# ldyken53/gaussian-splatting-wgpu

Hardware: AMD Instinct MI355X
Metric: frames/sec (higher is better)
Workload: dtype f32; 1 GPU; bicycle-like synthetic 6.1M gaussians @1920x1080; gaussians=6100000, width=1920, height=1080, tile_size=16, parallelism=single GPU, visible=2430918, processed=15909895, block_evaluated=6068168, sort_passes=1, depth_ordered_emission=True, tight_binning=True, blend_mode=fused, camera=64-step orbit, moved every frame

## Files before the change

### gaussian-splatting-wgpu_amd/csrc/k_blend.hip

```cpp
#include "gs_device.h"
#include "gs_tight.h"
#include <type_traits>

__device__ __forceinline__ float block_qmin(float cx, float cy, float cz, float dxlo, float dxhi, float dylo, float dyhi,
                                            float& mag) {
    const float X = __builtin_fminf(__builtin_fmaxf(0.0f, dxlo), dxhi);
    const float Y = __builtin_fminf(__builtin_fmaxf(0.0f, dylo), dyhi);
    float q = 3.0e38f;
    mag = 0.0f;
    if (X == 0.0f && Y == 0.0f) return 0.0f;
    if (X != 0.0f) {
        const float dy = __builtin_fminf(__builtin_fmaxf(-cy * X * __builtin_amdgcn_rcpf(cz), dylo), dyhi);
        const float a = 0.5f * cx * X * X, b = 0.5f * cz * dy * dy, c = cy * X * dy;
        q = a + b + c;
        mag = __builtin_fabsf(a) + __builtin_fabsf(b) + __builtin_fabsf(c);
    }
    if (Y != 0.0f) {
        const float dx = __builtin_fminf(__builtin_fmaxf(-cy * Y * __builtin_amdgcn_rcpf(cx), dxlo), dxhi);
        const float a = 0.5f * cx * dx * dx, b = 0.5f * cz * Y * Y, c = cy * dx * Y;
        const float q2 = a + b + c;
        if (q2 < q) { q = q2; mag = __builtin_fabsf(a) + __builtin_fabsf(b) + __builtin_fabsf(c); }
    }
    return q;
}

__device__ __forceinline__ bool blend_tmax_cull(float cx, float cy, float cz, float op, float dxlo, float dxhi, float dylo, float dyhi, float Tmax) {
    const float ax0 = (0.5f * cx) * dxlo * dxlo, ax1 = (0.5f * cx) * dxhi * dxhi, by0 = (0.5f * cz) * dylo * dylo, by1 = (0.5f * cz) * dyhi * dyhi;
    const float c00 = cy * dxlo * dylo, c01 = cy * dxlo * dyhi, c10 = cy * dxhi * dylo, c11 = cy * dxhi * dyhi;
    const float qmax = __builtin_fmaxf(__builtin_fmaxf(ax0 + by0 + c00, ax0 + by1 + c01), __builtin_fmaxf(ax1 + by0 + c10, ax1 + by1 + c11));
    const float qmag = __builtin_fmaxf(ax0, ax1) + __builtin_fmaxf(by0, by1) +
                       __builtin_fmaxf(__builtin_fmaxf(__builtin_fabsf(c00), __builtin_fabsf(c01)), __builtin_fmaxf(__builtin_fabsf(c10), __builtin_fabsf(c11)));
    const float alo = 0.99f * __builtin_fminf(0.99f, op * __builtin_amdgcn_exp2f(-1.44269502162933349609375f * (qmax + 1.0e-5f * qmag)));
    return Tmax * (1.0f - alo) < 0.0000999f;
}

struct GsAuxPlanes { float* alpha; float* depth; };
__device__ __forceinline__ GsAuxPlanes gs_aux_planes() { return GsAuxPlanes{nullptr, nullptr}; }
__device__ __forceinline__ GsAuxPlanes gs_aux_planes(GsAuxPlanes p) { return p; }

template <int TS, bool EXACT, bool AUX = false, typename... Aux>
__global__ __launch_bounds__(TS* TS) void gs_blend_kernel(const uint4* __restrict__ gdata, const uint32_t* __restrict__ values,
                                                           const uint32_t* __restrict__ ranges, GsFrame f,
                                                           uint32_t* __restrict__ rgba8, float* __restrict__ rgbf, GsControl* ctl,
                                                           uint32_t dbg, uint32_t id_mask, Aux... aux) {
    static_assert(sizeof...(Aux) == (AUX ? 1u : 0u), "AUX kernels take one GsAuxPlanes, the others none");
    constexpr int NT = TS * TS;
    constexpr int ROUNDS = NT / 64;
    constexpr int WPR = TS / 8;
    __shared__ float4 sP0[2][NT];
    __shared__ float4 sP1[2][NT];
    __shared__ float4 sP2[2][NT];

    const uint32_t tid = threadIdx.x, lane = tid & 63, w = tid >> 6;
    const uint32_t tx = f.col0 + blockIdx.x, ty = blockIdx.y;
    const uint32_t tile = tx + ty * f.ntx;
    const uint32_t start = tile > 0 ? ranges[tile - 1] : 0u;
    uint32_t end = ranges[tile];
    if (end > f.capacity) end = f.capacity;

    const uint32_t bx0 = tx * TS + (w % WPR) * 8, by0 = ty * TS + (w / WPR) * 8;
    const uint32_t gx = bx0 + (lane & 7), gy = by0 + (lane >> 3);
    const float pxf = (float)gx, pyf = (float)gy;
    const float bx0f = (float)bx0, by0f = (float)by0;
    float T = 1.0f, cr = 0.0f, cg = 0.0f, cb = 0.0f;
    float cd = 0.0f;
    const bool outside = !(gx < f.width && gy < f.height);
    bool done = outside;
    const float c255 = (float)(1.0 / 255.0);
    const float Wf = (float)f.width, Hf = (float)f.height;
    uint32_t staged = 0, evaluated = 0;

    const uint32_t piece = lane & 3u, qrec = lane >> 2;
    uint4 rq[4];
    uint32_t gnext = 0;
    auto fetch_ids = [&](uint32_t b) { gnext = (b + tid < end) ? values[b + tid] : 0u; };
    auto fetch = [&](uint32_t b, uint32_t gval) {
#pragma unroll
        for (int i = 0; i < 4; ++i) {
            const uint32_t rec = qrec + 16u * i;
            uint32_t g = __shfl(gval, rec, 64) & id_mask;
#ifdef GS_PROFILING
            if (dbg & 2u) g &= 1023u;
#endif
            if (b + w * 64u + rec < end && piece < 3u) rq[i] = gdata[(uint64_t)g * 4 + piece];
        }
    };
    auto stage = [&](uint32_t b, int buf) {
#pragma unroll
        for (int i = 0; i < 4; ++i) {
            const uint32_t e = w * 64u + qrec + 16u * i;
            if (b + e < end) {
                const float x = __uint_as_float(rq[i].x), y = __uint_as_float(rq[i].y), z = __uint_as_float(rq[i].z),
                            ww = __uint_as_float(rq[i].w);
                if (piece == 0u) {
                    sP0[buf][e].x = x * Wf;
                    sP0[buf][e].y = y * Hf;
                } else if (piece == 1u) {
                    const float L = 1.44269502162933349609375f;
                    sP1[buf][e] = EXACT ? make_float4(x, y, z, ww) : make_float4((-0.5f * L) * x, (-L) * y, (-0.5f * L) * z, ww);
                } else if (piece == 2u) {
                    sP2[buf][e] = make_float4(x, y, z, ww);
                    sP0[buf][e].z = __builtin_amdgcn_logf(ww * 255.0f) * 0.693147182464599609375f + 0.01f;
                }
            }
        }
    };

    uint32_t gcur = 0;
    if (start < end) {
        fetch_ids(start);
        gcur = gnext;
        fetch(start, gcur);
        fetch_ids(start + NT);
        stage(start, 0);
    }
    __syncthreads();
    int buf = 0;
    for (uint32_t b = start; b < end; b += NT, buf ^= 1) {
        const uint32_t nb = b + NT;
        if (nb < end) {
            gcur = gnext;
            fetch(nb, gcur);
            fetch_ids(nb + NT);
        }
        const uint32_t cnt = (end - b < (uint32_t)NT) ? end - b : (uint32_t)NT;
        staged += cnt;
        const unsigned long long lv = __ballot(!done);
        if (lv != 0ull) {
            uint32_t lcm = (uint32_t)lv | (uint32_t)(lv >> 32);
            lcm |= lcm >> 16; lcm |= lcm >> 8; lcm &= 0xFFu;
            const float lc0 = (float)__builtin_ctz(lcm | 0x100u), lc1 = (float)(31 - __builtin_clz(lcm | 1u));
            const float lr0 = (float)(__builtin_ctzll(lv) >> 3), lr1 = (float)((63 - __builtin_clzll(lv)) >> 3);
            const float Tmax = __uint_as_float((uint32_t)__builtin_amdgcn_readlane((int)wave_incl_max(done ? 0u : __float_as_uint(T)), 63));
#pragma unroll 1
            for (int r = 0; r < ROUNDS; ++r) {
                const uint32_t e0 = (uint32_t)r * 64u;
                if (e0 >= cnt) break;
                bool rel = false;
                if (e0 + lane < cnt) {
                    const float4 p0 = sP0[buf][e0 + lane];
                    float4 p1 = sP1[buf][e0 + lane];
                    if (!EXACT) {
                        const float iL = 0.693147182464599609375f;
                        p1.x *= -2.0f * iL;
                        p1.y *= -iL;
                        p1.z *= -2.0f * iL;
                    }
                    const float dxh = p0.x - bx0f, dyh = p0.y - by0f;
                    const float dxlo = dxh - lc1, dxhi = dxh - lc0, dylo = dyh - lr1, dyhi = dyh - lr0;
                    const bool pd = (p1.x > 0.0f) && (p1.z > 0.0f) && (p1.x * p1.z - p1.y * p1.y > 0.0f);
                    float mag;
                    const float q = block_qmin(p1.x, p1.y, p1.z, dxlo, dxhi, dylo, dyhi, mag);
                    const bool nocull = (dbg & 4u) != 0u;
                    rel = nocull || !pd || !(q > p0.z + 1.0e-5f * mag);
                    if (rel && pd && !nocull && blend_tmax_cull(p1.x, p1.y, p1.z, sP2[buf][e0 + lane].w, dxlo, dxhi, dylo, dyhi, Tmax)) rel = false;
#ifdef GS_PROFILING
                    if (dbg & 1u) rel = false;
#endif
                }
                unsigned long long m = __ballot(rel);
                evaluated += (uint32_t)__popcll(m);
                while (m) {
                    const uint32_t e = e0 + (uint32_t)__builtin_ctzll(m);
                    m &= m - 1ull;
                    const float4 p0 = sP0[buf][e];
                    const float4 p1 = sP1[buf][e];
                    const float4 p2v = sP2[buf][e];
                    const float dx = p0.x - pxf, dy = p0.y - pyf;
                    if (EXACT) {
                        const float t1 = p1.x * dx * dx, t2 = p1.z * dy * dy, t3 = p1.y * dx * dy;
                        const float power = -0.5f * (t1 + t2) - t3;
                        const float alpha = wg_min(0.99f, p2v.w * gs_exp(power));
                        const float test = T * (1.0f - alpha);
                        const float cond = (power <= 0.0f && alpha >= c255 && test >= 0.0001f) ? 1.0f : 0.0f;
                        cr += cond * p2v.x * alpha * T;
                        cg += cond * p2v.y * alpha * T;
                        cb += cond * p2v.z * alpha * T;
                        if constexpr (AUX) cd += cond * p1.w * alpha * T;
                        T = cond * test + (1.0f - cond) * T;
                    } else {
                        const float u = __builtin_fmaf(p1.x, dx, p1.y * dy);
                        const float v = (p1.z * dy) * dy;
                        const float pw = __builtin_fmaf(dx, u, v);
                        const float alpha = __builtin_fminf(0.99f, p2v.w * __builtin_amdgcn_exp2f(pw));
                        const float test = __builtin_fmaf(-T, alpha, T);
                        const bool keep = (pw <= 0.0f) && (alpha >= c255) && (test >= 0.0001f);
                        const float ak = keep ? alpha : 0.0f;
                        const float wgt = ak * T;
                        cr = __builtin_fmaf(p2v.x, wgt, cr);
                        cg = __builtin_fmaf(p2v.y, wgt, cg);
                        cb = __builtin_fmaf(p2v.z, wgt, cb);
                        if constexpr (AUX) cd = __builtin_fmaf(p1.w, wgt, cd);
                        T = keep ? test : T;
                    }
                }
            }
            if (EXACT) done = outside || (T * (1.0f - c255) < 0.0001f);
            else done = outside || (__builtin_fmaf(-T, c255, T) < 0.0001f);
        }
        if (nb < end) stage(nb, buf ^ 1);
        if (__syncthreads_and(done ? 1 : 0)) break;
    }
    if (tid == 0 && staged) atomicAdd(&ctl->num_processed[(blockIdx.x + blockIdx.y * gridDim.x) & 63u], (unsigned long long)staged);
    if (lane == 0 && evaluated) atomicAdd(&ctl->num_evaluated[(blockIdx.x + blockIdx.y * gridDim.x + w) & 63u], (unsigned long long)evaluated);

    if (!outside) {
        const float c[3] = {cr, cg, cb};
        uint32_t q = 0xFF000000u;
#pragma unroll
        for (int ch = 0; ch < 3; ++ch) {
            float v = c[ch];
            v = (v != v) ? 0.0f : wg_min(wg_max(v, 0.0f), 1.0f);
            q |= (uint32_t)__builtin_floorf(v * 255.0f + 0.5f) << (8 * ch);
        }
        const uint64_t o = (uint64_t)gy * f.slab_w + (gx - f.px0);
        rgba8[o] = q;
        if (rgbf) {
            rgbf[o * 3 + 0] = cr;
            rgbf[o * 3 + 1] = cg;
            rgbf[o * 3 + 2] = cb;
        }
        if constexpr (AUX) {
            const GsAuxPlanes ap = gs_aux_planes(aux...);
            ap.alpha[o] = 1.0f - T;
            ap.depth[o] = cd;
        }
    }
}

#ifdef GS_PROFILING
__device__ unsigned long long gs_blend_foot[256][16];
extern "C" __attribute__((visibility("default"))) int gs_prof_blend_footprint(unsigned long long* out4, int reset) {
    static unsigned long long h[256][16];
    if (out4) {
        if (hipMemcpyFromSymbol(h, HIP_SYMBOL(gs_blend_foot), sizeof(h)) != hipSuccess) return -1;
        for (int k = 0; k < 11; ++k) { out4[k] = 0; for (int c = 0; c < 256; ++c) out4[k] += h[c][k]; }
    }
    if (reset) { for (auto& r : h) for (auto& v : r) v = 0; if (hipMemcpyToSymbol(HIP_SYMBOL(gs_blend_foot), h, sizeof(h)) != hipSuccess) return -1; }
    return 0;
}
#endif
constexpr bool gs_lds_disjoint(int a, int na, int b, int nb) { return a + na <= b || b + nb <= a; }
typedef uint32_t gs_u32x2 __attribute__((ext_vector_type(2)));
typedef uint32_t gs_u32x3 __attribute__((ext_vector_type(3)));
typedef uint32_t gs_u32x4 __attribute__((ext_vector_type(4)));
template <bool EXACT, int TS = 16, bool MASKED = false, bool AUX = false, typename... Aux>
__global__ __launch_bounds__(64) void gs_blend_quad_kernel(const uint4* __restrict__ gdata, const uint32_t* __restrict__ values,
                                                            const uint32_t* __restrict__ ranges, GsFrame f,
                                                            uint32_t* __restrict__ rgba8, float* __restrict__ rgbf, GsControl* ctl,
                                                            uint32_t* __restrict__ tile_depth, uint32_t dbg, uint32_t* __restrict__ prof,
                                                            Aux... aux) {
    static_assert(sizeof...(Aux) == (AUX ? 1u : 0u), "AUX kernels take one GsAuxPlanes, the others none");
    constexpr uint32_t BPR = TS / 8, NB = BPR * BPR;
#ifdef GS_PROFILING
    const uint32_t t_start = prof ? (uint32_t)__builtin_amdgcn_s_memrealtime() : 0u;
#endif
#ifndef GS_L_OFF_T
#define GS_L_OFF_T 0
#define GS_L_OFF_Q 4160
#define GS_L_OFF_P 5184
#define GS_L_OFF_L 6208
#define GS_L_TOTAL 6464
#endif
#define GS_L_OFF_Z GS_L_TOTAL
#define GS_L_TOTAL_AUX (GS_L_TOTAL + 256)
    static_assert(gs_lds_disjoint(GS_L_OFF_T, 8 * 65 * 8, GS_L_OFF_Q, 256 * 4) && gs_lds_disjoint(GS_L_OFF_T, 8 * 65 * 8, GS_L_OFF_P, 64 * 16) &&
                  gs_lds_disjoint(GS_L_OFF_T, 8 * 65 * 8, GS_L_OFF_L, 64 * 4) && gs_lds_disjoint(GS_L_OFF_T, 8 * 65 * 8, GS_L_OFF_Z, 64 * 4) &&
                  gs_lds_disjoint(GS_L_OFF_Q, 256 * 4, GS_L_OFF_P, 64 * 16) && gs_lds_disjoint(GS_L_OFF_Q, 256 * 4, GS_L_OFF_L, 64 * 4) &&
                  gs_lds_disjoint(GS_L_OFF_Q, 256 * 4, GS_L_OFF_Z, 64 * 4) && gs_lds_disjoint(GS_L_OFF_P, 64 * 16, GS_L_OFF_L, 64 * 4) &&
                  gs_lds_disjoint(GS_L_OFF_P, 64 * 16, GS_L_OFF_Z, 64 * 4) && gs_lds_disjoint(GS_L_OFF_L, 64 * 4, GS_L_OFF_Z, 64 * 4),
                  "fused LDS regions overlap");
    static_assert(GS_L_OFF_T + 8 * 65 * 8 <= GS_L_TOTAL && GS_L_OFF_Q + 256 * 4 <= GS_L_TOTAL && GS_L_OFF_P + 64 * 16 <= GS_L_TOTAL &&
                  GS_L_OFF_L + 64 * 4 <= GS_L_TOTAL && GS_L_OFF_Z + 64 * 4 <= GS_L_TOTAL_AUX && GS_L_OFF_P % 16 == 0 && GS_L_OFF_T % 8 == 0,
                  "a fused LDS region ends outside its array");
    __shared__ __attribute__((aligned(16))) unsigned char lds_x[EXACT ? 4096 : 16];
    __shared__ __attribute__((aligned(16))) unsigned char lds_f[EXACT ? 16 : (AUX ? GS_L_TOTAL_AUX : GS_L_TOTAL)];
    float4* const sP0 = reinterpret_cast<float4*>(EXACT ? lds_x : lds_f + GS_L_OFF_P);
    float4* const sP1 = reinterpret_cast<float4*>(lds_x + (EXACT ? 1024 : 0));
    float4* const sP2 = reinterpret_cast<float4*>(lds_x + (EXACT ? 2048 : 0));
    uint32_t* const sQ = reinterpret_cast<uint32_t*>(EXACT ? lds_x + 3072 : lds_f + GS_L_OFF_Q);
    float* const sL = reinterpret_cast<float*>(lds_f + (EXACT ? 0 : GS_L_OFF_L));
    float2* const sT = reinterpret_cast<float2*>(lds_f + (EXACT ? 0 : GS_L_OFF_T));
    float* const sZ = reinterpret_cast<float*>(lds_f + ((EXACT || !AUX) ? 0 : GS_L_OFF_Z));
    const uint32_t lane = threadIdx.x;
    const uint32_t slab_tx = f.col1 - f.col0;
    const uint32_t b = blockIdx.x;
    const uint32_t x = b & 7u, j = b >> 3, q = j % NB, t = j / NB;
    const uint32_t SW = (dbg >> 8) & 0xffu;
    const uint32_t ns = (slab_tx + SW - 1) / SW;
    if (x >= ns) return;
    const uint32_t n_x = (ns - 1 - x) / 8 + 1;
    const uint32_t lastw = slab_tx - (ns - 1) * SW;
    const uint32_t Wx = n_x * SW - ((((ns - 1) & 7u) == x) ? SW - lastw : 0u);
    if (t >= Wx * f.nty) return;
    const uint32_t ty = t / Wx, cc = t % Wx;
    const uint32_t tx = f.col0 + (x + 8u * (cc / SW)) * SW + cc % SW;
    const uint32_t lin = ty * slab_tx + (tx - f.col0);
    const uint32_t tile = tx + ty * f.ntx;
    const uint32_t start = tile > 0 ? ranges[tile - 1] : 0u;
    uint32_t end = ranges[tile];
    if (end > f.capacity) end = f.capacity;
    const float c255 = (float)(1.0 / 255.0);
    const float Wf = (float)f.width, Hf = (float)f.height;
    const uint32_t bx0 = tx * TS + (q % BPR) * 8u, by0 = ty * TS + (q / BPR) * 8u;
    const uint32_t gx = bx0 + (lane & 7), gy = by0 + (lane >> 3);
    const float pxf = (float)gx, pyf = (float)gy, bx0f = (float)bx0, by0f = (float)by0;
    const bool outside = !(gx < f.width && gy < f.height);
    bool done = outside;
    float T = 1.0f, cr = 0.0f, cg = 0.0f, cb = 0.0f;
    float cd = 0.0f;
    uint32_t staged = 0, evaluated = 0;
#ifdef GS_PROFILING
    uint32_t fp_lanes = 0, fp_quads = 0, fp_none = 0, fp_live = 0, fp_kept = 0, fp_dead = 0, fp_q1 = 0, fp_tailn = 0, fp_tailbits = 0, fp_nokeep = 0;
#endif

    using R1 = std::conditional_t<AUX, gs_u32x4, gs_u32x3>;
    gs_u32x2 r0 = {0u, 0u};
    R1 r1 = {0u, 0u, 0u};
    gs_u32x4 r2 = {0u, 0u, 0u, 0u};
    const uint32_t mybit = GS_ID_BITS + (TS == 32 ? ((q / BPR) / 2u) * 2u + ((q % BPR) / 2u) : q);
    uint32_t qhead = 0, qn = 0;
    uint32_t pos = start;
    uint32_t g0 = 0, g1 = 0, g2 = 0;
    const __amdgpu_buffer_rsrc_t list_rsrc = __builtin_amdgcn_make_buffer_rsrc((void*)(values + start), 0, (int)((end - start) * 4u), 0x00020000);
    const uint32_t lane4 = lane * 4u;
    auto load_ids = [&]() {
        const uint32_t so = (pos - start) * 4u;
        g0 = __builtin_amdgcn_raw_buffer_load_b32(list_rsrc, lane4, so, 0);
        g1 = __builtin_amdgcn_raw_buffer_load_b32(list_rsrc, lane4 + 256u, so, 0);
        g2 = __builtin_amdgcn_raw_buffer_load_b32(list_rsrc, lane4 + 512u, so, 0);
    };
    const uint32_t mybitmask = 1u << mybit;
    auto push = [&](uint32_t v, uint32_t first) {
        bool want;
        if (MASKED) want = (v & mybitmask) != 0u;
        else want = first + lane < end;
        const unsigned long long m = __ballot(want);
        if (want) sQ[__builtin_amdgcn_mbcnt_hi((uint32_t)(m >> 32), __builtin_amdgcn_mbcnt_lo((uint32_t)m, qhead + qn)) & 255u] = v;
        qn += (uint32_t)__popcll(m);
    };
    auto fill = [&]() {
        while (qn < 64u && pos < end) {
            push(g0, pos); push(g1, pos + 64u); push(g2, pos + 128u);
            const uint32_t adv = end - pos < 192u ? end - pos : 192u;
            staged += adv;
            pos += adv;
            if (pos < end) load_ids();
        }
        __builtin_amdgcn_fence(__ATOMIC_RELEASE, "wavefront");
        __builtin_amdgcn_fence(__ATOMIC_ACQUIRE, "wavefront");
    };
    auto take = [&](uint32_t& v) -> uint32_t {
        const uint32_t cnt = qn < 64u ? qn : 64u;
        v = sQ[(qhead + lane) & 255u];
        qhead = (qhead + cnt) & 255u;
        qn -= cnt;
        return cnt;
    };
    auto fetch = [&](uint32_t v, uint32_t cnt) {
        uint32_t g = MASKED ? (v & GS_ID_MASK) : v;
#ifdef GS_PROFILING
        if (dbg & 2u) g &= 1023u;
#endif
        g = lane < cnt ? g : 0u;
        const uint32_t* rec = reinterpret_cast<const uint32_t*>(gdata + (uint64_t)g * 4);
        r0 = *reinterpret_cast<const gs_u32x2*>(rec);
        r1 = *reinterpret_cast<const R1*>(rec + 4);
        r2 = *reinterpret_cast<const gs_u32x4*>(rec + 8);
    };
    uint32_t cnt = 0, vnext = 0;
    if (start < end) {
        load_ids();
        fill();
        cnt = take(vnext);
        fetch(vnext, cnt);
    }
    while (cnt) {
        bool rel = false, npd = false;
        asm volatile("" : "+v"(r0), "+v"(r1), "+v"(r2));
        const float gxp = __uint_as_float(r0.x) * Wf, gyp = __uint_as_float(r0.y) * Hf;
        const float cx = __uint_as_float(r1.x), cy = __uint_as_float(r1.y), cz = __uint_as_float(r1.z);
        const float op = __uint_as_float(r2.w);
        float z = 0.0f;
        if constexpr (AUX) z = __uint_as_float(r1.w);
        const unsigned long long lv = __ballot(!done);
        uint32_t lcm = (uint32_t)lv | (uint32_t)(lv >> 32);
        lcm |= lcm >> 16; lcm |= lcm >> 8; lcm &= 0xFFu;
        const float lc0 = (float)__builtin_ctz(lcm | 0x100u), lc1 = (float)(31 - __builtin_clz(lcm | 1u));
        const float lr0 = (float)(__builtin_ctzll(lv | (1ull << 63)) >> 3), lr1 = (float)((63 - __builtin_clzll(lv | 1ull)) >> 3);
        const float Tmax = __uint_as_float((uint32_t)__builtin_amdgcn_readlane((int)wave_incl_max(done ? 0u : __float_as_uint(T)), 63));
        if (lane < cnt) {
            const float lim = __builtin_amdgcn_logf(op * 255.0f) * 0.693147182464599609375f + 0.01f;
            const bool pd = (cx > 0.0f) && (cz > 0.0f) && (cx * cz - cy * cy > 0.0f);
            {
                const float dxh = gxp - bx0f, dyh = gyp - by0f;
                float mag;
                const float qm = block_qmin(cx, cy, cz, dxh - lc1, dxh - lc0, dyh - lr1, dyh - lr0, mag);
                const bool nocull = (dbg & 4u) != 0u;
                rel = lv != 0ull && (nocull || !pd || !(qm > lim + 1.0e-5f * mag));
#ifndef GS_NO_TMAX
                if (rel && pd && !nocull) {
                    const float x0 = dxh - lc1, x1 = dxh - lc0, y0 = dyh - lr1, y1 = dyh - lr0;
                    const float ax0 = (0.5f * cx) * x0 * x0, ax1 = (0.5f * cx) * x1 * x1, by0 = (0.5f * cz) * y0 * y0, by1 = (0.5f * cz) * y1 * y1;
                    const float c00 = cy * x0 * y0, c01 = cy * x0 * y1, c10 = cy * x1 * y0, c11 = cy * x1 * y1;
                    const float qmax = __builtin_fmaxf(__builtin_fmaxf(ax0 + by0 + c00, ax0 + by1 + c01), __builtin_fmaxf(ax1 + by0 + c10, ax1 + by1 + c11));
                    const float qmag = __builtin_fmaxf(ax0, ax1) + __builtin_fmaxf(by0, by1) +
                                       __builtin_fmaxf(__builtin_fmaxf(__builtin_fabsf(c00), __builtin_fabsf(c01)), __builtin_fmaxf(__builtin_fabsf(c10), __builtin_fabsf(c11)));
                    const float alo = 0.99f * __builtin_fminf(0.99f, op * __builtin_amdgcn_exp2f(-1.44269502162933349609375f * (qmax + 1.0e-5f * qmag)));
                    if (Tmax * (1.0f - alo) < 0.0000999f) rel = false;
                }
#endif
#ifdef GS_BLEND_PIXTEST
                if (rel && pd && !nocull && (uint32_t)__popcll(lv) <= GS_BLEND_PIXTEST) {
                    bool any = false;
                    for (unsigned long long mm = lv; mm; mm &= mm - 1ull) {
                        const int pl = __builtin_ctzll(mm);
                        const float Tp = __uint_as_float((uint32_t)__builtin_amdgcn_readlane((int)__float_as_uint(T), pl));
                        const float dx = dxh - (float)(pl & 7), dy = dyh - (float)(pl >> 3);
                        const float a = (0.5f * cx) * dx * dx, b = (0.5f * cz) * dy * dy, c = cy * dx * dy;
                        const float q = a + b + c, mg = 1.0e-5f * (a + b + __builtin_fabsf(c));
                        const float ahi = 1.01f * (op * __builtin_amdgcn_exp2f(-1.44269502162933349609375f * (q - mg)));
                        const float alo = 0.99f * __builtin_fminf(0.99f, op * __builtin_amdgcn_exp2f(-1.44269502162933349609375f * (q + mg)));
                        any = any || !(ahi < c255 || Tp * (1.0f - alo) < 0.0000999f);
                    }
                    rel = any;
                }
#endif
            }
#ifdef GS_PROFILING
            if (dbg & 1u) rel = false;
#endif
            npd = rel && !pd;
        }
#ifdef GS_PROFILING
        if ((dbg & 32u) && MASKED && __popcll(lv) <= 16) {
            const unsigned long long rm = __ballot(rel);
            const uint32_t bits = __popc((vnext >> GS_ID_BITS) & 15u);
            fp_tailn += (uint32_t)__popcll(rm);
            fp_tailbits += (uint32_t)__popcll(__ballot(rel && bits >= 1u)) + (uint32_t)__popcll(__ballot(rel && bits >= 2u)) + (uint32_t)__popcll(__ballot(rel && bits >= 3u)) + (uint32_t)__popcll(__ballot(rel && bits >= 4u));
        }
#endif
        const unsigned long long m = __ballot(rel);
        if (rel) {
            const uint32_t slot = __builtin_amdgcn_mbcnt_hi((uint32_t)(m >> 32), __builtin_amdgcn_mbcnt_lo((uint32_t)m, 0u));
            const float L = 1.44269502162933349609375f;
            if (EXACT) {
                sP0[slot] = make_float4(gxp, gyp, 0.0f, 0.0f);
                sP1[slot] = make_float4(cx, cy, cz, z);
                sP2[slot] = make_float4(__uint_as_float(r2.x), __uint_as_float(r2.y), __uint_as_float(r2.z), op);
            } else {
                const float hx = (-0.5f * L) * cx, hy = (-L) * cy, hz = (-0.5f * L) * cz;
                const float lop = __builtin_amdgcn_logf(op) + 0.014499569695115089f;
                const float d = gxp - bx0f;
                const float b0 = (-2.0f * hx) * d, a1 = hy * d, a0 = __builtin_fmaf(hx * d, d, lop);
                sP0[slot] = make_float4(hx, 0.99f * __uint_as_float(r2.x), 0.99f * __uint_as_float(r2.y), 0.99f * __uint_as_float(r2.z));
                sL[slot] = lop;
                if constexpr (AUX) sZ[slot] = 0.99f * z;
#pragma unroll
                for (int r = 0; r < 8; ++r) {
                    const float dy = gyp - (by0f + (float)r);
                    sT[r * 65 + slot] = make_float2(__builtin_fmaf(-hy, dy, b0), __builtin_fmaf(dy, __builtin_fmaf(dy, hz, a1), a0));
                }
            }
        }
        fill();
        const uint32_t cnt_next = take(vnext);
        if (cnt_next) fetch(vnext, cnt_next);
        __builtin_amdgcn_fence(__ATOMIC_RELEASE, "wavefront");
        __builtin_amdgcn_fence(__ATOMIC_ACQUIRE, "wavefront");
        const uint32_t nrel = (uint32_t)__popcll(m);
        evaluated += nrel;
        const uint32_t trow = (lane >> 3) * 65u;
        const float xlf = (float)(lane & 7u);
        auto walk = [&](auto checked_tag) {
            constexpr bool CHECKED = decltype(checked_tag)::value;
            auto one = [&](uint32_t e, const float4 p0, const float2 tt, const float zz) {
                if (EXACT) {
                    const float dx = p0.x - pxf;
                    const float4 p1 = sP1[e];
                    const float dy = p0.y - pyf;
                    const float4 p2v = sP2[e];
                    const float t1 = p1.x * dx * dx, t2 = p1.z * dy * dy, t3 = p1.y * dx * dy;
                    const float power = -0.5f * (t1 + t2) - t3;
                    const float alpha = wg_min(0.99f, p2v.w * gs_exp(power));
                    const float test = T * (1.0f - alpha);
                    const float cond = (power <= 0.0f && alpha >= c255 && test >= 0.0001f) ? 1.0f : 0.0f;
                    cr += cond * p2v.x * alpha * T;
                    cg += cond * p2v.y * alpha * T;
                    cb += cond * p2v.z * alpha * T;
                    if constexpr (AUX) cd += cond * p1.w * alpha * T;
                    T = cond * test + (1.0f - cond) * T;
                } else {
                    const float pw = __builtin_fmaf(xlf, __builtin_fmaf(xlf, p0.x, tt.x), tt.y);
                    float ea;
                    asm("v_exp_f32_e64 %0, %1 clamp" : "=v"(ea) : "v"(pw));
                    const float k1 = (float)(1.0 / 255.0 / 0.99);
#ifdef GS_PROFILING
                    if (dbg & 32u) {
                        const unsigned long long km = __ballot(ea >= k1);
                        const unsigned long long q0 = 0x000000000F0F0F0Full;
                        fp_lanes += (uint32_t)__popcll(km);
                        fp_quads += (uint32_t)((km & q0) != 0) + (uint32_t)((km & (q0 << 4)) != 0) + (uint32_t)((km & (q0 << 32)) != 0) + (uint32_t)((km & (q0 << 36)) != 0);
                        fp_none += (uint32_t)(km == 0);
                        const unsigned long long lv = __ballot(__builtin_fmaf(-T, c255, T) >= 0.0001f);
                        const unsigned long long kp = __ballot(ea >= k1 && __builtin_fmaf(T * ea, -0.99f, T) >= 0.0001f);
                        fp_live += (uint32_t)__popcll(lv);
                        fp_kept += (uint32_t)__popcll(kp);
                        fp_dead += (uint32_t)((km & lv) == 0);
                        fp_q1 += (uint32_t)(__popcll(lv) <= 16);
                        fp_nokeep += (uint32_t)(kp == 0ull);
                    }
#endif
                    if (CHECKED) {
                        const float wgt = T * ea;
                        const float test = __builtin_fmaf(wgt, -0.99f, T);
                        bool keep = (ea >= k1) && (test >= 0.0001f);
                        keep = keep && (pw <= sL[e]);
                        const float wk = keep ? wgt : 0.0f;
                        cr = __builtin_fmaf(p0.y, wk, cr);
                        cg = __builtin_fmaf(p0.z, wk, cg);
                        cb = __builtin_fmaf(p0.w, wk, cb);
                        if constexpr (AUX) cd = __builtin_fmaf(zz, wk, cd);
                        T = keep ? test : T;
                    } else {
                        float wgt, test;
                        unsigned long long save;
                        if constexpr (AUX)
                            asm(
                                "v_mul_f32_e32 %[wgt], %[T], %[ea]\n\t"
                                "v_fma_f32 %[test], %[wgt], %[m99], %[T]\n\t"
                                "s_mov_b64 %[save], exec\n\t"
                                "v_cmpx_le_f32_e32 vcc, %[k1], %[ea]\n\t"
                                "v_cmpx_le_f32_e32 vcc, %[thr], %[test]\n\t"
                                "v_mov_b32_e32 %[T], %[test]\n\t"
                                "v_fmac_f32_e32 %[cr], %[c0], %[wgt]\n\t"
                                "v_fmac_f32_e32 %[cg], %[c1], %[wgt]\n\t"
                                "v_fmac_f32_e32 %[cb], %[c2], %[wgt]\n\t"
                                "v_fmac_f32_e32 %[cd], %[z], %[wgt]\n\t"
                                "s_mov_b64 exec, %[save]"
                                : [save] "=&s"(save), [wgt] "=&v"(wgt), [test] "=&v"(test), [T] "+v"(T), [cr] "+v"(cr), [cg] "+v"(cg), [cb] "+v"(cb),
                                  [cd] "+v"(cd)
                                : [k1] "s"(k1), [thr] "s"(0.0001f), [m99] "s"(-0.99f), [ea] "v"(ea), [c0] "v"(p0.y), [c1] "v"(p0.z), [c2] "v"(p0.w),
                                  [z] "v"(zz)
                                : "vcc");
                        else
                        asm(
                            "v_mul_f32_e32 %[wgt], %[T], %[ea]\n\t"
                            "v_fma_f32 %[test], %[wgt], %[m99], %[T]\n\t"
                            "s_mov_b64 %[save], exec\n\t"
                            "v_cmpx_le_f32_e32 vcc, %[k1], %[ea]\n\t"
                            "v_cmpx_le_f32_e32 vcc, %[thr], %[test]\n\t"
                            "v_mov_b32_e32 %[T], %[test]\n\t"
                            "v_fmac_f32_e32 %[cr], %[c0], %[wgt]\n\t"
                            "v_fmac_f32_e32 %[cg], %[c1], %[wgt]\n\t"
                            "v_fmac_f32_e32 %[cb], %[c2], %[wgt]\n\t"
                            "s_mov_b64 exec, %[save]"
                            : [save] "=&s"(save), [wgt] "=&v"(wgt), [test] "=&v"(test), [T] "+v"(T), [cr] "+v"(cr), [cg] "+v"(cg), [cb] "+v"(cb)
                            : [k1] "s"(k1), [thr] "s"(0.0001f), [m99] "s"(-0.99f), [ea] "v"(ea), [c0] "v"(p0.y), [c1] "v"(p0.z), [c2] "v"(p0.w)
                            : "vcc");
                    }
                }
            };
            auto group = [&](uint32_t e, auto n_tag) {
                constexpr int G = decltype(n_tag)::value;
                float4 p[G];
                float2 t[G];
                float zz[G];
#pragma unroll
                for (int k = 0; k < G; ++k) {
                    p[k] = sP0[e + k];
                    t[k] = EXACT ? make_float2(0.0f, 0.0f) : sT[trow + e + k];
                    zz[k] = 0.0f;
                    if constexpr (AUX && !EXACT) zz[k] = sZ[e + k];
                }
                __builtin_amdgcn_sched_barrier(0);
#pragma unroll
                for (int k = 0; k < G; ++k) one(e + k, p[k], t[k], zz[k]);
                __builtin_amdgcn_sched_barrier(0);
            };
            uint32_t e = 0;
            if (!EXACT)
                for (; e + 8u <= nrel; e += 8u) group(e, std::integral_constant<int, 8>{});
            for (; e + 4u <= nrel; e += 4u) group(e, std::integral_constant<int, 4>{});
            for (; e < nrel; ++e) group(e, std::integral_constant<int, 1>{});
        };
        if (EXACT || __ballot(npd) != 0ull) walk(std::true_type{});
        else walk(std::false_type{});
        if (EXACT) done = outside || (T * (1.0f - c255) < 0.0001f);
        else done = outside || (__builtin_fmaf(-T, c255, T) < 0.0001f);
        __builtin_amdgcn_fence(__ATOMIC_RELEASE, "wavefront");
        __builtin_amdgcn_fence(__ATOMIC_ACQUIRE, "wavefront");
        if (__ballot(!done) == 0ull) break;
        cnt = cnt_next;
    }
    if (lane == 0 && staged) atomicMax(&tile_depth[lin], staged);
    if (lane == 0 && evaluated) atomicAdd(&ctl->num_evaluated[(b + 1u) & 63u], (unsigned long long)evaluated);
#ifdef GS_PROFILING
    if ((dbg & 32u) && lane == 0) {
        unsigned long long* fp = gs_blend_foot[b & 255u];
        atomicAdd(&fp[0], (unsigned long long)evaluated); atomicAdd(&fp[1], (unsigned long long)fp_lanes);
        atomicAdd(&fp[2], (unsigned long long)fp_quads); atomicAdd(&fp[3], (unsigned long long)fp_none);
        atomicAdd(&fp[4], (unsigned long long)fp_live); atomicAdd(&fp[5], (unsigned long long)fp_kept);
        atomicAdd(&fp[6], (unsigned long long)fp_dead); atomicAdd(&fp[7], (unsigned long long)fp_q1);
        atomicAdd(&fp[8], (unsigned long long)fp_tailn); atomicAdd(&fp[9], (unsigned long long)fp_tailbits); atomicAdd(&fp[10], (unsigned long long)fp_nokeep);
    }
    if (prof && lane == 0) {
        prof[b * 4u + 0u] = t_start;
        prof[b * 4u + 1u] = (uint32_t)__builtin_amdgcn_s_memrealtime();
        prof[b * 4u + 2u] = evaluated;
        prof[b * 4u + 3u] = staged;
    }
#endif
    if (!outside) {
        const float c[3] = {cr, cg, cb};
        uint32_t px = 0xFF000000u;
#pragma unroll
        for (int ch = 0; ch < 3; ++ch) {
            float v = c[ch];
            v = (v != v) ? 0.0f : wg_min(wg_max(v, 0.0f), 1.0f);
            px |= (uint32_t)__builtin_floorf(v * 255.0f + 0.5f) << (8 * ch);
        }
        const uint64_t o = (uint64_t)gy * f.slab_w + (gx - f.px0);
        rgba8[o] = px;
        if (rgbf) {
            rgbf[o * 3 + 0] = cr;
            rgbf[o * 3 + 1] = cg;
            rgbf[o * 3 + 2] = cb;
        }
        if constexpr (AUX) {
            const GsAuxPlanes ap = gs_aux_planes(aux...);
            ap.alpha[o] = 1.0f - T;
            ap.depth[o] = cd;
        }
    }
}

__global__ __launch_bounds__(256) void gs_assemble_kernel(const uint32_t* __restrict__ slabs, uint32_t* __restrict__ image,
                                                           uint32_t width, uint32_t height, const uint32_t* __restrict__ px_bounds,
                                                           uint32_t n_slabs, uint64_t slab_stride_px) {
    const uint64_t t = (uint64_t)blockIdx.x * 256 + threadIdx.x;
    if (t >= (uint64_t)width * height) return;
    const uint32_t y = (uint32_t)(t / width), x = (uint32_t)(t % width);
    uint32_t g = 0;
    while (g + 1 < n_slabs && x >= px_bounds[g + 1]) ++g;
    const uint32_t x0 = px_bounds[g], w = px_bounds[g + 1] - x0;
    const uint64_t slab_off = slab_stride_px ? (uint64_t)g * slab_stride_px : (uint64_t)x0 * height;
    image[t] = slabs[slab_off + (uint64_t)y * w + (x - x0)];
}

__global__ __launch_bounds__(256) void gs_debug_view_kernel(const uint32_t* __restrict__ ranges, GsFrame f, uint32_t view,
                                                             uint32_t* __restrict__ rgba8) {
    const uint64_t t = (uint64_t)blockIdx.x * 256 + threadIdx.x;
    if (t >= (uint64_t)f.slab_w * f.height) return;
    const uint32_t y = (uint32_t)(t / f.slab_w), x = f.px0 + (uint32_t)(t % f.slab_w);
    const uint32_t tile = x / f.tile_size + (y / f.tile_size) * f.ntx;
    const uint32_t start = tile > 0 ? ranges[tile - 1] : 0u, end = ranges[tile];
    const float len = (float)(end - start);
    float c[3];
    if (view == 1u) {
        if (x % f.tile_size != f.tile_size - 1u && y % f.tile_size != f.tile_size - 1u) return;
        c[0] = 1.0f; c[1] = 0.0f; c[2] = 0.0f;
    } else if (view == 2u) {
        c[0] = c[1] = c[2] = len / 1000.0f;
    } else if (view == 3u) {
        c[0] = (float)x / (float)f.width; c[1] = (float)y / (float)f.height; c[2] = 0.0f;
    } else {
        c[0] = c[1] = len / 100.0f; c[2] = 0.0f;
    }
    uint32_t px = 0xFF000000u;
#pragma unroll
    for (int ch = 0; ch < 3; ++ch) {
        const float v = wg_min(wg_max(c[ch], 0.0f), 1.0f);
        px |= (uint32_t)__builtin_floorf(v * 255.0f + 0.5f) << (8 * ch);
    }
    rgba8[t] = px;
}
void gs_launch_debug_view(const uint32_t* ranges, const GsFrame& f, uint32_t view, uint32_t* rgba8, hipStream_t st) {
    const uint64_t total = (uint64_t)f.slab_w * f.height;
    if (!total || !view) return;
    hipLaunchKernelGGL(gs_debug_view_kernel, dim3((uint32_t)((total + 255) / 256)), dim3(256), 0, st, ranges, f, view, rgba8);
}

template <int TS>
static void launch_blend_t(bool exact, bool aux, GsAuxPlanes ap, dim3 grid, hipStream_t st, const uint4* gdata, const uint32_t* values,
                           const uint32_t* ranges, const GsFrame& f, uint32_t* rgba8, float* rgbf, GsControl* ctl, uint32_t dbg, uint32_t id_mask) {
#define GS_WG(E) hipLaunchKernelGGL((gs_blend_kernel<TS, E>), grid, dim3(TS * TS), 0, st, gdata, values, ranges, f, rgba8, rgbf, ctl, dbg, id_mask)
#define GS_WG_AUX(E) hipLaunchKernelGGL((gs_blend_kernel<TS, E, true, GsAuxPlanes>), grid, dim3(TS * TS), 0, st, gdata, values, ranges, f, rgba8, \
                                        rgbf, ctl, dbg, id_mask, ap)
    if (aux) { if (exact) GS_WG_AUX(true); else GS_WG_AUX(false); }
    else { if (exact) GS_WG(true); else GS_WG(false); }
#undef GS_WG
#undef GS_WG_AUX
}
template <int TS>
static void launch_quad_t(bool exact, bool masked, bool aux, GsAuxPlanes ap, uint32_t nblk, uint32_t pad, hipStream_t st, const uint4* g,
                          const uint32_t* values, const uint32_t* ranges, const GsFrame& f, uint32_t* rgba8, float* rgbf, GsControl* ctl,
                          uint32_t* tile_depth, uint32_t dbg, uint32_t* prof) {
#define GS_QUAD(E, M) hipLaunchKernelGGL((gs_blend_quad_kernel<E, TS, M>), dim3(nblk), dim3(64), pad, st, g, values, ranges, f, rgba8, rgbf, ctl, tile_depth, dbg, prof)
#define GS_QUAD_AUX(E, M) hipLaunchKernelGGL((gs_blend_quad_kernel<E, TS, M, true, GsAuxPlanes>), dim3(nblk), dim3(64), pad, st, g, values, ranges, f, \
                                             rgba8, rgbf, ctl, tile_depth, dbg, prof, ap)
    if (aux) {
        if (exact) { if (masked) GS_QUAD_AUX(true, true); else GS_QUAD_AUX(true, false); }
        else { if (masked) GS_QUAD_AUX(false, true); else GS_QUAD_AUX(false, false); }
    } else {
        if (exact) { if (masked) GS_QUAD(true, true); else GS_QUAD(true, false); }
        else { if (masked) GS_QUAD(false, true); else GS_QUAD(false, false); }
    }
#undef GS_QUAD
#undef GS_QUAD_AUX
}
int gs_launch_blend(const void* gdata, const uint32_t* values, const uint32_t* ranges, const GsFrame& f, uint32_t* rgba8, float* rgbf,
                    bool aux, float* alpha, float* depth, GsControl* ctl, uint32_t* tile_depth, bool exact, uint32_t ablation, bool masked,
                    hipStream_t st, uint32_t* prof, uint32_t* prof_blocks) {
    if (aux && (!alpha || !depth)) return -2;
    const GsAuxPlanes ap{alpha, depth};
    uint32_t dbg = ablation;
    const uint32_t id_mask = masked ? GS_ID_MASK : 0xFFFFFFFFu;
    const dim3 grid(f.col1 - f.col0, f.nty);
    if (grid.x == 0 || grid.y == 0) return 1;
    const uint4* g = (const uint4*)gdata;
    switch (f.tile_size) {
    case 8: launch_blend_t<8>(exact, aux, ap, grid, st, g, values, ranges, f, rgba8, rgbf, ctl, dbg, id_mask); return 1;
    case 16:
    case 32: {
        const bool t32 = f.tile_size == 32;
        if (!(dbg & 8u)) {
            const uint32_t slab_tx = grid.x;
            auto widest = [&](uint32_t sw) {
                const uint32_t ns = (slab_tx + sw - 1) / sw, lastw = slab_tx - (ns - 1) * sw;
                uint32_t wmax = 0;
                for (uint32_t x = 0; x < 8 && x < ns; ++x) {
                    const uint32_t n_x = (ns - 1 - x) / 8 + 1, wx = n_x * sw - ((((ns - 1) & 7u) == x) ? sw - lastw : 0u);
                    wmax = wx > wmax ? wx : wmax;
                }
                return wmax;
            };
            uint32_t SW = (dbg >> 8) & 0xffu;
            if (!SW) {
                SW = 1;
                for (uint32_t sw = 3; sw > 1; --sw)
                    if (widest(sw) * 80u <= slab_tx * 11u) { SW = sw; break; }
            }
            dbg = (dbg & 0xffu) | (SW << 8);
            const uint32_t wmax = widest(SW);
            const uint32_t nblk = (t32 ? 128u : 32u) * wmax * grid.y;
#ifdef GS_PROFILING
            const uint32_t pad = (dbg & 64u) ? 20480u - 3072u : (dbg & 128u) ? 10240u - 3072u : 0u;
#else
            const uint32_t pad = 0u;
#endif
            if (prof_blocks) *prof_blocks = nblk;
            if (t32) { launch_quad_t<32>(exact, masked, aux, ap, nblk, pad, st, g, values, ranges, f, rgba8, rgbf, ctl, tile_depth, dbg, prof); return 16; }
            launch_quad_t<16>(exact, masked, aux, ap, nblk, pad, st, g, values, ranges, f, rgba8, rgbf, ctl, tile_depth, dbg, prof);
            return 4;
        }
        if (t32) { launch_blend_t<32>(exact, aux, ap, grid, st, g, values, ranges, f, rgba8, rgbf, ctl, dbg, id_mask); return 1; }
        launch_blend_t<16>(exact, aux, ap, grid, st, g, values, ranges, f, rgba8, rgbf, ctl, dbg, id_mask);
        return 1;
    }
    default: return -1;
    }
}
void gs_launch_assemble(const void* slabs, void* image, uint32_t width, uint32_t height, const uint32_t* d_px_bounds, uint32_t n_slabs,
                        uint64_t slab_stride_px, hipStream_t st) {
    const uint64_t total = (uint64_t)width * height;
    hipLaunchKernelGGL(gs_assemble_kernel, dim3((uint32_t)((total + 255) / 256)), dim3(256), 0, st, (const uint32_t*)slabs, (uint32_t*)image,
                       width, height, d_px_bounds, n_slabs, slab_stride_px);
}
```

### gaussian-splatting-wgpu_amd/gsplat/_abi.py

```python
import ctypes
import os

import numpy as np

_HERE = os.path.dirname(os.path.abspath(__file__))
LIB_PATH = os.environ.get("GSPLAT_LIB") or os.path.abspath(os.path.join(_HERE, "..", "lib", "libgsplat_hip.so"))

GS_FLAG_EXACT_BLEND = 0x1
GS_FLAG_F32_TAP = 0x2
GS_FLAG_TIMING = 0x4
GS_FLAG_AUX_OUTPUTS = 0x8

GS_STAGE_NAMES = ("preprocess", "scan", "emit", "sort", "ranges", "blend")

(GS_BUF_TILE_COUNTS, GS_BUF_TILE_OFFSETS, GS_BUF_GAUSSIAN_DATA, GS_BUF_KEYS_UNSORTED, GS_BUF_VALUES_UNSORTED, GS_BUF_KEYS,
 GS_BUF_VALUES, GS_BUF_RANGES, GS_BUF_RGBA8, GS_BUF_RGB_F32, GS_BUF_BLOCK_MASKS) = range(11)
GS_BUF_ALPHA_F32 = 13
GS_BUF_DEPTH_F32 = 14

GS_OPT_BLEND_ABLATION = 1
GS_OPT_PERSISTENT_GRID = 2
GS_OPT_RESET_TIMING = 3
GS_OPT_EMIT_ORDER = 4
GS_OPT_UNFUSED = 5
GS_OPT_DEBUG_VIEW = 6
GS_OPT_TILE_CULL = 7
GS_OPT_FRAMES_IN_FLIGHT = 8
GS_OPT_FRAME_GRAPH = 9
GS_OPT_PROJ_CHUNKS = 10

GS_ERR_INVALID_ARGUMENT = -1
GS_ERR_NO_FRAME = -6

GS_PICK_OK = 0
GS_PICK_OUTSIDE_SLAB = 1
GS_PICK_NONE = 0xFFFFFFFF
GS_PICK_MAX_QUERIES = 65536
GS_PICK_MAX_CONTRIB = 256

ABI_SYMBOLS = ("gs_last_error", "gs_abi_version", "gs_create", "gs_destroy", "gs_upload_splats", "gs_upload_splats_device",
               "gs_share_splats",
               "gs_ply_load", "gs_ply_free", "gs_upload_ply",
               "gs_render", "gs_render_debug", "gs_render_to", "gs_wait", "gs_render_host", "gs_wait_ticket", "gs_host_alloc", "gs_host_free", "gs_read_rgba8", "gs_read_buffer", "gs_device_ptr",
               "gs_get_stats", "gs_pick", "gs_set_option", "gs_slab_width", "gs_assemble_slabs", "gs_sort_pairs_u32",
               "gs_exclusive_scan_u32")


class GsConfig(ctypes.Structure):
    _fields_ = [("struct_size", ctypes.c_uint32), ("width", ctypes.c_uint32), ("height", ctypes.c_uint32),
                ("tile_size", ctypes.c_uint32), ("device", ctypes.c_int32), ("col_begin", ctypes.c_uint32),
                ("col_end", ctypes.c_uint32), ("flags", ctypes.c_uint32), ("max_intersections", ctypes.c_uint64),
                ("stream", ctypes.c_void_p)]


class GsStats(ctypes.Structure):
    _fields_ = [("num_gaussians", ctypes.c_uint64), ("num_visible", ctypes.c_uint64), ("num_intersections", ctypes.c_uint64),
                ("num_processed", ctypes.c_uint64), ("num_tiles", ctypes.c_uint32), ("sort_passes", ctypes.c_uint32),
                ("frames", ctypes.c_uint64), ("stage_us", ctypes.c_float * 6), ("frame_us", ctypes.c_float),
                ("stage_us_mean", ctypes.c_float * 6), ("frame_us_mean", ctypes.c_float), ("frames_timed", ctypes.c_uint32), ("depth_ordered", ctypes.c_uint32), ("num_evaluated", ctypes.c_uint64),
                ("capacity", ctypes.c_uint64), ("max_intersections_seen", ctypes.c_uint64), ("truncated_frames", ctypes.c_uint64),
                ("tight_binning", ctypes.c_uint32), ("frames_in_flight", ctypes.c_uint32), ("graph_frames", ctypes.c_uint64),
                ("num_row_items", ctypes.c_uint64), ("num_row_slots", ctypes.c_uint64), ("row_capacity", ctypes.c_uint64)]


class GsPickQuery(ctypes.Structure):
    _fields_ = [("x", ctypes.c_uint32), ("y", ctypes.c_uint32)]


class GsPickResult(ctypes.Structure):
    _fields_ = [("status", ctypes.c_uint32), ("list_length", ctypes.c_uint32), ("hit_count", ctypes.c_uint32),
                ("first_id", ctypes.c_uint32), ("first_depth", ctypes.c_float), ("max_id", ctypes.c_uint32),
                ("max_weight", ctypes.c_float), ("median_id", ctypes.c_uint32), ("median_depth", ctypes.c_float),
                ("alpha", ctypes.c_float), ("depth_acc", ctypes.c_float), ("reserved", ctypes.c_uint32)]


class GsPickContrib(ctypes.Structure):
    _fields_ = [("id", ctypes.c_uint32), ("weight", ctypes.c_float)]


PICK_RESULT_DTYPE = np.dtype([(n, np.float32 if t is ctypes.c_float else np.uint32) for n, t in GsPickResult._fields_])
PICK_CONTRIB_DTYPE = np.dtype([("id", np.uint32), ("weight", np.float32)])


class GsError(RuntimeError):
    def __init__(self, code, msg):
        super().__init__("gsplat error %d: %s" % (code, msg))
        self.code = code


_lib = None


def load():
    global _lib
    if _lib is not None:
        return _lib
    if not os.path.exists(LIB_PATH):
        raise ImportError("libgsplat_hip.so not built: run `python gaussian-splatting-wgpu_amd/csrc/build.py` "
                          "(or __graft_entry__.build()); there is no CPU fallback")
    L = ctypes.CDLL(LIB_PATH)
    vp, u64, i32, u32 = ctypes.c_void_p, ctypes.c_uint64, ctypes.c_int32, ctypes.c_uint32
    L.gs_last_error.restype = ctypes.c_char_p
    L.gs_abi_version.restype = i32
    L.gs_create.argtypes = [ctypes.POINTER(GsConfig), ctypes.POINTER(vp)]
    L.gs_destroy.argtypes = [vp]
    L.gs_upload_splats.argtypes = [vp, vp, u64]
    L.gs_upload_splats_device.argtypes = [vp, vp, u64]
    L.gs_share_splats.argtypes = [vp, vp]
    L.gs_ply_load.argtypes = [ctypes.c_char_p, ctypes.POINTER(vp), ctypes.POINTER(u64), ctypes.POINTER(i32)]
    L.gs_ply_free.argtypes = [vp]
    L.gs_upload_ply.argtypes = [vp, ctypes.c_char_p, ctypes.POINTER(u64)]
    L.gs_render.argtypes = [vp, vp]
    L.gs_render_debug.argtypes = [vp, vp]
    L.gs_render_to.argtypes = [vp, vp, vp]
    L.gs_wait.argtypes = [vp]
    L.gs_render_host.argtypes = [vp, vp, vp, u64, ctypes.POINTER(u64)]
    L.gs_wait_ticket.argtypes = [vp, u64]
    L.gs_host_alloc.argtypes = [u64, ctypes.POINTER(vp)]
    L.gs_host_free.argtypes = [vp]
    L.gs_read_rgba8.argtypes = [vp, vp, u64]
    L.gs_read_buffer.argtypes = [vp, i32, vp, u64, ctypes.POINTER(u64)]
    L.gs_device_ptr.argtypes = [vp, i32, ctypes.POINTER(vp)]
    L.gs_get_stats.argtypes = [vp, ctypes.POINTER(GsStats)]
    L.gs_pick.argtypes = [vp, vp, u32, vp, u32, vp]
    L.gs_set_option.argtypes = [vp, i32, ctypes.c_int64]
    L.gs_slab_width.argtypes = [vp, ctypes.POINTER(u32), ctypes.POINTER(u32)]
    L.gs_assemble_slabs.argtypes = [vp, vp, ctypes.POINTER(u32), u32, u64, vp]
    L.gs_sort_pairs_u32.argtypes = [i32, vp, vp, u64, u32]
    L.gs_exclusive_scan_u32.argtypes = [i32, vp, u64, ctypes.POINTER(u64)]
    for name in ABI_SYMBOLS:
        if name not in ("gs_last_error", "gs_ply_free", "gs_host_free"):
            getattr(L, name).restype = i32
    L.gs_ply_free.restype = None
    L.gs_host_free.restype = None
    _lib = L
    return L


def check(rc):
    if rc != 0:
        raise GsError(rc, load().gs_last_error().decode("utf-8", "replace"))


def sort_pairs(keys, values=None, key_bits=32, device=0):
    k = np.array(keys, dtype=np.uint32, copy=True)
    v = None if values is None else np.array(values, dtype=np.uint32, copy=True)
    check(load().gs_sort_pairs_u32(device, k.ctypes.data, None if v is None else v.ctypes.data, k.size, key_bits))
    return k, v


def exclusive_scan(data, device=0):
    d = np.array(data, dtype=np.uint32, copy=True)
    total = ctypes.c_uint64(0)
    check(load().gs_exclusive_scan_u32(device, d.ctypes.data, d.size, ctypes.byref(total)))
    return d, int(total.value)


def load_ply(path):
    L = load()
    rec, n, deg = ctypes.c_void_p(), ctypes.c_uint64(), ctypes.c_int32()
    check(L.gs_ply_load(str(path).encode(), ctypes.byref(rec), ctypes.byref(n), ctypes.byref(deg)))
    try:
        arr = np.ctypeslib.as_array(ctypes.cast(rec, ctypes.POINTER(ctypes.c_float)), shape=(max(n.value, 1) * 80,))[: n.value * 80]
        return arr.reshape(n.value, 80).copy(), deg.value
    finally:
        L.gs_ply_free(rec)
```

Before: 1341 frames/s.

## Add few-live-pixel fast path in blend that iterates over surviving pixels

When six or fewer pixels in the 8x8 block are still live and every gaussian in the batch has a positive-definite conic, the blend kernel leaves the usual cull/Tmax/grouped walk. Instead it loops over each live pixel, evaluates all batch gaussians for that pixel in parallel across lanes, and then serially composites the ones that pass using readlane broadcasts. This is meant to avoid the per-batch culling and walk overhead when almost all pixels in the block have saturated. In exchange it adds serialized per-pixel and per-contributor loops with readlanes, which can cost more if many gaussians contribute, and a different evaluation order that may change precision slightly.

```diff
diff --git a/gaussian-splatting-wgpu_amd/csrc/k_blend.hip b/gaussian-splatting-wgpu_amd/csrc/k_blend.hip
--- a/gaussian-splatting-wgpu_amd/csrc/k_blend.hip
+++ b/gaussian-splatting-wgpu_amd/csrc/k_blend.hip
@@ -240,6 +240,32 @@
     return 0;
 }
 #endif
+#ifdef GS_PROFILING
+__device__ unsigned long long gs_blend_fewlive_hist[64][18][4];
+extern "C" __attribute__((visibility("default"))) int gs_prof_blend_fewlive(unsigned long long* out72, int reset) {
+    static unsigned long long h[64][18][4];
+    if (out72) {
+        if (hipMemcpyFromSymbol(h, HIP_SYMBOL(gs_blend_fewlive_hist), sizeof(h)) != hipSuccess) return -1;
+        for (int k = 0; k < 72; ++k) { out72[k] = 0; for (int c = 0; c < 64; ++c) out72[k] += h[c][k / 4][k % 4]; }
+    }
+    if (reset) { for (auto& c : h) for (auto& r : c) for (auto& v : r) v = 0; if (hipMemcpyToSymbol(HIP_SYMBOL(gs_blend_fewlive_hist), h, sizeof(h)) != hipSuccess) return -1; }
+    return 0;
+}
+#endif
+#ifndef GS_BLEND_FEWLIVE
+#define GS_BLEND_FEWLIVE 6
+#endif
+#define GS_BLEND_KEEP_ASM                             \
+    "v_mul_f32_e32 %[wgt], %[T], %[ea]\n\t"           \
+    "v_fma_f32 %[test], %[wgt], %[m99], %[T]\n\t"     \
+    "s_mov_b64 %[save], exec\n\t"                     \
+    "v_cmpx_le_f32_e32 vcc, %[k1], %[ea]\n\t"         \
+    "v_cmpx_le_f32_e32 vcc, %[thr], %[test]\n\t"      \
+    "v_mov_b32_e32 %[T], %[test]\n\t"                 \
+    "v_fmac_f32_e32 %[cr], %[c0], %[wgt]\n\t"         \
+    "v_fmac_f32_e32 %[cg], %[c1], %[wgt]\n\t"         \
+    "v_fmac_f32_e32 %[cb], %[c2], %[wgt]\n\t"         \
+    "s_mov_b64 exec, %[save]"
 constexpr bool gs_lds_disjoint(int a, int na, int b, int nb) { return a + na <= b || b + nb <= a; }
 typedef uint32_t gs_u32x2 __attribute__((ext_vector_type(2)));
 typedef uint32_t gs_u32x3 __attribute__((ext_vector_type(3)));
@@ -384,12 +410,43 @@
         float z = 0.0f;
         if constexpr (AUX) z = __uint_as_float(r1.w);
         const unsigned long long lv = __ballot(!done);
+#ifdef GS_PROFILING
+        auto hist = [&](uint32_t parked) {
+            if (!EXACT && (dbg & 32u) && lane == 0) {
+                const uint32_t nl = (uint32_t)__popcll(lv);
+                unsigned long long* h = gs_blend_fewlive_hist[b & 63u][nl < 17u ? nl : 17u];
+                atomicAdd(&h[0], 1ull); atomicAdd(&h[1], (unsigned long long)cnt); atomicAdd(&h[2], (unsigned long long)parked);
+                if (!parked) atomicAdd(&h[3], 1ull);
+            }
+        };
+#endif
+        bool few = false;
+        float hx = 0.0f, hy = 0.0f, hz = 0.0f, b0 = 0.0f, a1 = 0.0f, a0 = 0.0f, c0 = 0.0f, c1 = 0.0f, c2 = 0.0f;
+        if constexpr (!EXACT && !AUX) {
+            few = (dbg & (4u | 16u)) == 0u && (uint32_t)__popcll(lv) <= (uint32_t)GS_BLEND_FEWLIVE;
+#ifdef GS_PROFILING
+            few = few && !(dbg & 1u);
+#endif
+            if (few) {
+                const float det = cx * cz - cy * cy;
+                const bool sound = (cx > 0.0f) && (cz > 0.0f) && (det > 0.0f) && (det < __builtin_inff());
+                few = __ballot(lane < cnt && !sound) == 0ull;
+            }
+            if (few) {
+                const float L = 1.44269502162933349609375f;
+                hx = (-0.5f * L) * cx, hy = (-L) * cy, hz = (-0.5f * L) * cz;
+                const float lop = __builtin_amdgcn_logf(op) + 0.014499569695115089f;
+                const float d = gxp - bx0f;
+                b0 = (-2.0f * hx) * d, a1 = hy * d, a0 = __builtin_fmaf(hx * d, d, lop);
+                c0 = 0.99f * __uint_as_float(r2.x), c1 = 0.99f * __uint_as_float(r2.y), c2 = 0.99f * __uint_as_float(r2.z);
+            }
+        }
         uint32_t lcm = (uint32_t)lv | (uint32_t)(lv >> 32);
         lcm |= lcm >> 16; lcm |= lcm >> 8; lcm &= 0xFFu;
         const float lc0 = (float)__builtin_ctz(lcm | 0x100u), lc1 = (float)(31 - __builtin_clz(lcm | 1u));
         const float lr0 = (float)(__builtin_ctzll(lv | (1ull << 63)) >> 3), lr1 = (float)((63 - __builtin_clzll(lv | 1ull)) >> 3);
-        const float Tmax = __uint_as_float((uint32_t)__builtin_amdgcn_readlane((int)wave_incl_max(done ? 0u : __float_as_uint(T)), 63));
-        if (lane < cnt) {
+        const float Tmax = few ? 0.0f : __uint_as_float((uint32_t)__builtin_amdgcn_readlane((int)wave_incl_max(done ? 0u : __float_as_uint(T)), 63));
+        if (!few && lane < cnt) {
             const float lim = __builtin_amdgcn_logf(op * 255.0f) * 0.693147182464599609375f + 0.01f;
             const bool pd = (cx > 0.0f) && (cz > 0.0f) && (cx * cz - cy * cy > 0.0f);
             {
@@ -544,17 +601,7 @@
                                   [z] "v"(zz)
                                 : "vcc");
                         else
-                        asm(
-                            "v_mul_f32_e32 %[wgt], %[T], %[ea]\n\t"
-                            "v_fma_f32 %[test], %[wgt], %[m99], %[T]\n\t"
-                            "s_mov_b64 %[save], exec\n\t"
-                            "v_cmpx_le_f32_e32 vcc, %[k1], %[ea]\n\t"
-                            "v_cmpx_le_f32_e32 vcc, %[thr], %[test]\n\t"
-                            "v_mov_b32_e32 %[T], %[test]\n\t"
-                            "v_fmac_f32_e32 %[cr], %[c0], %[wgt]\n\t"
-                            "v_fmac_f32_e32 %[cg], %[c1], %[wgt]\n\t"
-                            "v_fmac_f32_e32 %[cb], %[c2], %[wgt]\n\t"
-                            "s_mov_b64 exec, %[save]"
+                        asm(GS_BLEND_KEEP_ASM
                             : [save] "=&s"(save), [wgt] "=&v"(wgt), [test] "=&v"(test), [T] "+v"(T), [cr] "+v"(cr), [cg] "+v"(cg), [cb] "+v"(cb)
                             : [k1] "s"(k1), [thr] "s"(0.0001f), [m99] "s"(-0.99f), [ea] "v"(ea), [c0] "v"(p0.y), [c1] "v"(p0.z), [c2] "v"(p0.w)
                             : "vcc");
@@ -584,8 +631,52 @@
             for (; e + 4u <= nrel; e += 4u) group(e, std::integral_constant<int, 4>{});
             for (; e < nrel; ++e) group(e, std::integral_constant<int, 1>{});
         };
-        if (EXACT || __ballot(npd) != 0ull) walk(std::true_type{});
-        else walk(std::false_type{});
+        uint32_t nreached = 0;
+        if constexpr (!EXACT && !AUX) {
+            if (few) {
+                const bool have = lane < cnt;
+                const float k1 = (float)(1.0 / 255.0 / 0.99);
+                unsigned long long reached = 0ull;
+#pragma unroll 1
+                for (unsigned long long pm = lv; pm; pm &= pm - 1ull) {
+                    const uint32_t pl = (uint32_t)__builtin_ctzll(pm);
+                    const float xl = (float)(pl & 7u);
+                    const float dy = gyp - (by0f + (float)(pl >> 3));
+                    const float B = __builtin_fmaf(-hy, dy, b0), A = __builtin_fmaf(dy, __builtin_fmaf(dy, hz, a1), a0);
+                    const float pw = __builtin_fmaf(xl, __builtin_fmaf(xl, hx, B), A);
+                    float ea;
+                    asm("v_exp_f32_e64 %0, %1 clamp" : "=v"(ea) : "v"(pw));
+                    const float Tp = __uint_as_float((uint32_t)__builtin_amdgcn_readlane((int)__float_as_uint(T), (int)pl));
+                    unsigned long long cm = __ballot(have && ea >= k1 && __builtin_fmaf(Tp * ea, -0.99f, Tp) >= 0.0000999f);
+                    reached |= cm;
+#pragma unroll 1
+                    for (; cm; cm &= cm - 1ull) {
+                        const int cl = __builtin_ctzll(cm);
+                        const float ea1 = __uint_as_float((uint32_t)__builtin_amdgcn_readlane((int)__float_as_uint(ea), cl));
+                        const float q0 = __uint_as_float((uint32_t)__builtin_amdgcn_readlane((int)__float_as_uint(c0), cl));
+                        const float q1 = __uint_as_float((uint32_t)__builtin_amdgcn_readlane((int)__float_as_uint(c1), cl));
+                        const float q2 = __uint_as_float((uint32_t)__builtin_amdgcn_readlane((int)__float_as_uint(c2), cl));
+                        if (lane == pl) {
+                            float wgt, test;
+                            unsigned long long save;
+                            asm(GS_BLEND_KEEP_ASM
+                                : [save] "=&s"(save), [wgt] "=&v"(wgt), [test] "=&v"(test), [T] "+v"(T), [cr] "+v"(cr), [cg] "+v"(cg), [cb] "+v"(cb)
+                                : [k1] "s"(k1), [thr] "s"(0.0001f), [m99] "s"(-0.99f), [ea] "v"(ea1), [c0] "v"(q0), [c1] "v"(q1), [c2] "v"(q2)
+                                : "vcc");
+                        }
+                    }
+                }
+                nreached = (uint32_t)__popcll(reached);
+                evaluated += nreached;
+            }
+        }
+#ifdef GS_PROFILING
+        hist(nrel + nreached);
+#endif
+        if (!few) {
+            if (EXACT || __ballot(npd) != 0ull) walk(std::true_type{});
+            else walk(std::false_type{});
+        }
         if (EXACT) done = outside || (T * (1.0f - c255) < 0.0001f);
         else done = outside || (__builtin_fmaf(-T, c255, T) < 0.0001f);
         __builtin_amdgcn_fence(__ATOMIC_RELEASE, "wavefront");
diff --git a/gaussian-splatting-wgpu_amd/gsplat/_abi.py b/gaussian-splatting-wgpu_amd/gsplat/_abi.py
--- a/gaussian-splatting-wgpu_amd/gsplat/_abi.py
+++ b/gaussian-splatting-wgpu_amd/gsplat/_abi.py
@@ -19,6 +19,8 @@
 GS_BUF_DEPTH_F32 = 14
 
 GS_OPT_BLEND_ABLATION = 1
+GS_BLEND_ABLATION_NO_CULLS = 4
+GS_BLEND_ABLATION_NO_FEWLIVE = 16
 GS_OPT_PERSISTENT_GRID = 2
 GS_OPT_RESET_TIMING = 3
 GS_OPT_EMIT_ORDER = 4
```

New measurement: 1284 frames/s. 0.957x the previous value.
